# praateekmahajan/moving-mnist-vae

Hardware: AMD Instinct MI355X
Metric: frames/sec/GPU VAE train step, 20×64×64 batch; ELBO vs CPU ref (higher is better)
Workload: dtype bf16; 1 GPU; BASELINE configs[1]: 256 clips x 20 frames x 64x64 per GPU per step (=5120 frames), conv-VAE z=128, Gaussian NLL sigma=0.1 + KL (normal_vae_1_kl_0_mmd), Adam, random-init weights, Bernoulli(0.0521) q=2 labels; parallelism=dp1, rccl_ranks=1, grad_exchange=none, bn=per-rank batch statistics

## Files before the change

include/mmvae.h:

```cpp
#ifndef MMVAE_H_
#define MMVAE_H_

#include <stddef.h>
#include <stdint.h>

#ifdef __cplusplus
extern "C" {
#endif

#if defined(__GNUC__)
#define MMVAE_API __attribute__((visibility("default")))
#else
#define MMVAE_API
#endif

#define MMVAE_OK 0
#define MMVAE_ERR_ARG (-1)
#define MMVAE_ERR_HIP (-2)
#define MMVAE_ERR_WORKSPACE (-3)
#define MMVAE_ERR_UNSUPPORTED (-4)

#define MMVAE_F32 0
#define MMVAE_BF16 1
#define MMVAE_FP8 2
// ... 15 lines not shown
                    int32_t* kind, int64_t* offset);
MMVAE_API size_t mmvae_net_workspace_bytes(mmvae_net* net, int N);

MMVAE_API int mmvae_encoder_fwd(mmvae_net* net, int N, const float* x, const float* params, float* bn_f32, int64_t* bn_i64,
                      void* workspace, size_t workspace_bytes, float* mu, float* logvar, int training, void* stream);
MMVAE_API int mmvae_net_stage_labels(mmvae_net* net, int N, const void* labels, int label_bytes, float mean, float stdv, float* image,
                           void* workspace, size_t workspace_bytes, void* stream);
MMVAE_API int mmvae_encoder_fwd_staged(mmvae_net* net, int N, const float* x, const float* params, float* bn_f32, int64_t* bn_i64,
                             void* workspace, size_t workspace_bytes, float* mu, float* logvar, int training, void* stream);
MMVAE_API int mmvae_encoder_bwd(mmvae_net* net, int N, const float* d_mu, const float* d_logvar, const float* params, float* grads,
                      void* workspace, size_t workspace_bytes, void* stream);
MMVAE_API int mmvae_decoder_fwd(mmvae_net* net, int N, const float* encoding, const float* params, float* bn_f32, int64_t* bn_i64,
                      void* workspace, size_t workspace_bytes, float* recon, int training, void* stream);
MMVAE_API int mmvae_decoder_bwd(mmvae_net* net, int N, const float* d_recon, const float* params, float* grads, void* workspace,
                      size_t workspace_bytes, float* d_encoding , void* stream);
MMVAE_API int mmvae_decoder_bwd_gauss(mmvae_net* net, int N, const float* target, float sigma, float coef, const float* gscale, const float* params,
                            float* grads, void* workspace, size_t workspace_bytes, float* d_enc, void* stream);

MMVAE_API int mmvae_net_defer_join(mmvae_net* net, int enable);
MMVAE_API int mmvae_net_join(mmvae_net* net, void* stream);
MMVAE_API void* mmvae_net_fork(mmvae_net* net, void* stream);
MMVAE_API void* mmvae_net_side_stream(mmvae_net* net);
MMVAE_API int mmvae_net_set_join_grad(mmvae_net* net, int enable);

typedef int (*mmvae_allreduce_fn)(float* buf, int64_t n, void* stream, void* user);
MMVAE_API int mmvae_net_set_sync_bn(mmvae_net* net, mmvae_allreduce_fn fn, void* user, int world);

typedef struct mmvae_comm mmvae_comm;
#define MMVAE_COMM_ID_BYTES 128
MMVAE_API int mmvae_comm_unique_id(void* id_host );
MMVAE_API int mmvae_comm_init(mmvae_comm** out, int world, int rank, const void* id_host);
MMVAE_API int mmvae_comm_allreduce(mmvae_comm* comm, float* buf, int64_t n, void* stream);
MMVAE_API int mmvae_comm_destroy(mmvae_comm* comm);
MMVAE_API int mmvae_net_set_sync_bn_comm(mmvae_net* net, mmvae_comm* comm);
MMVAE_API int mmvae_net_set_sync_bn_comm2(mmvae_net* net, mmvae_comm* comm_main, mmvae_comm* comm_side);

MMVAE_API int mmvae_rsample_fwd(const float* mu, const float* logvar, const float* eps, float* enc, int64_t n, void* stream);
MMVAE_API int mmvae_rsample_bwd(const float* d_enc, const float* logvar, const float* eps, float* d_mu, float* d_logvar, int64_t n,
                      void* stream);
#define MMVAE_SUM_PARTIALS 1025
MMVAE_API int mmvae_kl_fwd(const float* mu, const float* logvar, int64_t n, double* acc, void* stream);
MMVAE_API int mmvae_kl_fwd_ex(const float* mu, const float* logvar, int64_t n, double* acc, double* partials, void* stream);
MMVAE_API int mmvae_kl_bwd(const float* mu, const float* logvar, float coef, const float* gscale, float* d_mu, float* d_logvar, int64_t n,
                 void* stream);
MMVAE_API int mmvae_gauss_nll_fwd(const float* recon, const float* target, int64_t n, float sigma, double* acc, void* stream);
MMVAE_API int mmvae_gauss_nll_fwd_ex(const float* recon, const float* target, int64_t n, float sigma, double* acc, double* partials,
// ... 79 lines not shown
MMVAE_API int mmvae_adam_step(float* params, const float* grads, float* exp_avg, float* exp_avg_sq, int64_t n, float lr, float beta1,
                    float beta2, float eps, float weight_decay, float bc1, float bc2_sqrt, float grad_scale, void* stream);

MMVAE_API int mmvae_adam_step_dev(float* params, const float* grads, float* exp_avg, float* exp_avg_sq, int64_t n, float lr, float beta1,
                        float beta2, float eps, float weight_decay, double* step_dev, float grad_scale, void* stream);

MMVAE_API int mmvae_grad_norm_sq(const float* grads, int64_t n, float grad_scale, double* acc, double* partials, void* stream);

MMVAE_API int mmvae_adam_step_guarded(float* params, const float* grads, float* exp_avg, float* exp_avg_sq, int64_t n, float lr, float beta1,
                            float beta2, float eps, float weight_decay, double* state, double* partials, float grad_scale,
                            float max_norm, void* stream);

MMVAE_API int mmvae_conv2d_fwd(int dtype, int transposed, const void* x, const float* weight, void* y, int N, int H, int W, int Cin, int Cout,
                     int k, int stride, int pad, const float* pro_scale, const float* pro_shift, int pro_relu, float* stats,
                     void* scratch, void* stream);
MMVAE_API int mmvae_conv2d_dgrad(int dtype, int transposed, const void* dy, const float* weight, void* dx, int N, int H, int W, int Cin,
                       int Cout, int k, int stride, int pad, void* scratch, void* stream);
#define MMVAE_DGRAD_EX_W2_OFFSET(numel_w, esize) ((((size_t)(numel_w) * (esize) + 255) / 256) * 256)
#define MMVAE_DGRAD_EX_SCRATCH_BYTES(numel_w, numel_w2, esize) \
  ((numel_w2) > 0 ? MMVAE_DGRAD_EX_W2_OFFSET(numel_w, esize) + (size_t)(numel_w2) * (esize) : (size_t)(numel_w) * (esize))
MMVAE_API int mmvae_conv2d_dgrad_ex(int dtype, int transposed, const void* dy, const float* weight, void* dx, int N, int H, int W, int Cin,
                          int Cout, int k, int stride, int pad, int accumulate, const void* dy2, const float* w2, int C2, void* scratch,
                          void* stream);
#define MMVAE_WGRAD_SCRATCH_BYTES (64u << 20)
MMVAE_API int mmvae_conv2d_wgrad(int dtype, int transposed, const void* x, const void* dy, float* dweight, int N, int H, int W, int Cin,
                       int Cout, int k, int stride, int pad, const float* pro_scale, const float* pro_shift, int pro_relu,
                       void* scratch, void* stream);
MMVAE_API int mmvae_conv2d_wgrad_pair(int dtype, const void* x, const void* dy, const void* dy_shortcut, float* dweight, float* dweight_sc, int N,
                            int H, int W, int Cin, int Cout, const float* pro_scale, const float* pro_shift, int pro_relu, void* scratch,
                            void* stream);
#define MMVAE_BN_SCRATCH_BYTES (16u << 20)
MMVAE_API int mmvae_batchnorm_fwd(int dtype, const void* y, int64_t npix, int C, const float* gamma, const float* beta, float* running_mean,
                        float* running_var, int64_t* nbt, float momentum, float eps, int relu, void* out, float* save_mean, float* save_istd,
                        void* scratch, void* stream);
MMVAE_API int mmvae_batchnorm_bwd(int dtype, const void* dout, const void* y, const void* out, int64_t npix, int C, const float* gamma,
                        const float* save_mean, const float* save_istd, void* dy, float* dgamma, float* dbeta, void* scratch, void* stream);
#define MMVAE_STEM_SCRATCH_BYTES 12800u
MMVAE_API int mmvae_stem_fwd(int dtype, const void* x, const float* weight, void* y, int N, int S, float* stats, void* scratch, void* stream);
MMVAE_API int mmvae_stem_bwd(int dtype, const void* g, const void* y0, const void* x, const float* weight, const float* gamma,
                   const float* bn_scale, const float* bn_shift, const float* save_mean, const float* save_istd, float* dweight,
                   float* dgamma, float* dbeta, int N, int S, void* scratch, void* stream);
MMVAE_API int mmvae_convT_bwd_fused(int dtype, const void* x, const void* dy, const float* weight, float* dweight, void* dx, int N, int H, int W,
                          int Cin, int Cout, int k, int stride, int pad, const float* pro_scale, const float* pro_shift, int pro_relu,
                          const void* x2, const float* w2, float* dw2, void* scratch, void* wscratch, void* stream);
MMVAE_API int mmvae_tail_join_fwd(int dtype, const void* y2, const float* s2, const float* b2, const void* ys, const float* ss, const float* bs,
                        const float* weight, const float* bias, float* r_raw, float* stats, int N, int H, int W, void* stream);
// ... 50 lines not shown
```

moving-mnist-vae_amd/_lib.py:

```python
from __future__ import annotations

import ctypes
import os
from ctypes import POINTER, c_char_p, c_double, c_float, c_int, c_int32, c_int64, c_size_t, c_uint64, c_void_p

import torch

_HERE = os.path.dirname(os.path.abspath(__file__))
LIB_PATH = os.environ.get("MMVAE_LIB_PATH") or os.path.join(_HERE, "libmmvae_hip.so")
_lib = None
ABI_VERSION = 3
SUM_PARTIALS = 1025
BN_SCRATCH_BYTES = 16 << 20
STEM_SCRATCH_BYTES = 12800

P = c_void_p

PROTOTYPES = {
    "mmvae_abi_version": (c_int, []),
    "mmvae_last_error": (c_char_p, []),
    "mmvae_net_create": (c_int, [POINTER(c_void_p), c_int, c_int, c_int, c_int, c_int, c_int]),
    "mmvae_net_create_ex": (c_int, [POINTER(c_void_p), c_int, c_int, c_int, c_int, c_int, c_int, c_int]),
    "mmvae_net_destroy": (None, [P]),
    "mmvae_net_sizes": (c_int, [P, POINTER(c_int64), POINTER(c_int64), POINTER(c_int32), POINTER(c_int64), POINTER(c_int32)]),
    "mmvae_net_num_entries": (c_int, [P]),
    "mmvae_net_entry": (c_int, [P, c_int, c_char_p, c_int, POINTER(c_int32), POINTER(c_int32), POINTER(c_int32), POINTER(c_int64)]),
    "mmvae_net_workspace_bytes": (c_size_t, [P, c_int]),
    "mmvae_encoder_fwd": (c_int, [P, c_int, P, P, P, P, P, c_size_t, P, P, c_int, P]),
    "mmvae_net_stage_labels": (c_int, [P, c_int, P, c_int, c_float, c_float, P, P, c_size_t, P]),
    "mmvae_encoder_fwd_staged": (c_int, [P, c_int, P, P, P, P, P, c_size_t, P, P, c_int, P]),
    "mmvae_encoder_bwd": (c_int, [P, c_int, P, P, P, P, P, c_size_t, P]),
    "mmvae_decoder_fwd": (c_int, [P, c_int, P, P, P, P, P, c_size_t, P, c_int, P]),
    "mmvae_decoder_bwd": (c_int, [P, c_int, P, P, P, P, c_size_t, P, P]),
    "mmvae_decoder_bwd_gauss": (c_int, [P, c_int, P, c_float, c_float, P, P, P, P, c_size_t, P, P]),
    "mmvae_net_defer_join": (c_int, [P, c_int]),
    "mmvae_net_join": (c_int, [P, P]),
    "mmvae_net_fork": (P, [P, P]),
    "mmvae_net_side_stream": (P, [P]),
    "mmvae_net_set_join_grad": (c_int, [P, c_int]),
    "mmvae_net_set_sync_bn": (c_int, [P, P, P, c_int]),
    "mmvae_rsample_fwd": (c_int, [P, P, P, P, c_int64, P]),
    "mmvae_rsample_bwd": (c_int, [P, P, P, P, P, c_int64, P]),
    "mmvae_kl_fwd": (c_int, [P, P, c_int64, P, P]),
    "mmvae_kl_fwd_ex": (c_int, [P, P, c_int64, P, P, P]),
    "mmvae_kl_bwd": (c_int, [P, P, c_float, P, P, P, c_int64, P]),
    "mmvae_gauss_nll_fwd": (c_int, [P, P, c_int64, c_float, P, P]),
    "mmvae_gauss_nll_fwd_ex": (c_int, [P, P, c_int64, c_float, P, P, P]),
    "mmvae_gauss_nll_bwd": (c_int, [P, P, c_int64, c_float, c_float, P, P, P]),
    "mmvae_ce_fwd": (c_int, [P, P, P, c_int, c_int, c_int, P, P]),
    "mmvae_ce_fwd_ex": (c_int, [P, P, P, c_int, c_int, c_int, P, P, P]),
    "mmvae_ce_bwd": (c_int, [P, P, P, c_int, c_int, c_int, c_float, P, P, P]),
    "mmvae_mmd_fwd": (c_int, [P, P, c_int, c_int, P, P, P]),
    "mmvae_mmd_fwd_ex": (c_int, [P, P, c_int, c_int, P, P, P, P]),
    "mmvae_mmd_bwd": (c_int, [P, P, c_int, c_int, c_float, P, P, P]),
    "mmvae_loss_finish": (c_int, [P, P, c_float, c_float, c_float, c_float, P]),
    "mmvae_gauss_nll_per_image": (c_int, [P, P, c_int, c_int64, c_float, P, P]),
    "mmvae_ce_per_image": (c_int, [P, P, P, c_int, c_int, c_int, P, P]),
    "mmvae_kl_per_image": (c_int, [P, P, c_int, c_int, P, P]),
    "mmvae_latent_logratio": (c_int, [P, P, P, c_int, c_int, P, P]),
    "mmvae_iw_bound": (c_int, [P, P, c_int, c_int, P, P]),
    "mmvae_normalise_labels": (c_int, [P, c_int64, c_float, c_float, P, P]),
    "mmvae_quantise_normalise": (c_int, [P, c_int64, P, c_int, c_float, c_float, P, P, P]),
    "mmvae_u8_histogram": (c_int, [P, c_int64, P, c_int64, P, P]),
    "mmvae_kmeans1d_fit": (c_int, [P, c_int, P, P]),
    "mmvae_quantiser_stats": (c_int, [P, P, c_int, P, P, P, P]),
    "mmvae_resample_coeffs": (c_int, [c_int, c_int, POINTER(c_int), P, P]),
    "mmvae_resize_quantise_normalise": (c_int, [P, c_int64, P, c_int, c_int64, c_int, c_int, c_int, c_int, P, P, c_int, P, P, c_int, P, c_int,
                                                c_float, c_float, P, P, P, P]),
    "mmvae_generate_clips": (c_int, [P, c_int64, c_int, P, c_uint64, c_int64, c_int64, c_int, c_int, c_int, P, c_int, c_float, c_float, P, P, P, P]),
    "mmvae_logits_to_labels": (c_int, [P, c_int, c_int, c_int, c_int, P, P, P]),
    "mmvae_panel_sheet": (c_int, [P, c_int, c_int, c_int, P, P]),
    "mmvae_scatter_panel": (c_int, [P, c_int64, c_int, c_int, c_int, P, c_int, c_int, P, P, c_int64, P]),
    "mmvae_latent_stats": (c_int, [P, P, P, c_int, c_int, c_int, P, P]),
    "mmvae_nearest_frames_scratch_bytes": (c_size_t, [c_int, c_int64, c_int, c_int]),
    "mmvae_nearest_frames": (c_int, [P, c_int, P, c_int64, c_int, P, c_int, P, P, P, c_size_t, P]),
    "mmvae_tensor_hist_chunks": (c_int64, [P, c_int, c_int64, P, c_int64]),
    "mmvae_tensor_hist_scratch_bytes": (c_size_t, [c_int, c_int64]),
    "mmvae_tensor_hist": (c_int, [P, c_int64, P, P, c_int, P, P, c_int64, P, P, P, P, P, c_size_t, P]),
    "mmvae_adam_step": (c_int, [P, P, P, P, c_int64, c_float, c_float, c_float, c_float, c_float, c_float, c_float, c_float, P]),
    "mmvae_adam_step_dev": (c_int, [P, P, P, P, c_int64, c_float, c_float, c_float, c_float, c_float, P, c_float, P]),
    "mmvae_grad_norm_sq": (c_int, [P, c_int64, c_float, P, P, P]),
    "mmvae_adam_step_guarded": (c_int, [P, P, P, P, c_int64, c_float, c_float, c_float, c_float, c_float, P, P, c_float, c_float, P]),
    "mmvae_conv2d_fwd": (c_int, [c_int, c_int, P, P, P, c_int, c_int, c_int, c_int, c_int, c_int, c_int, c_int, P, P, c_int, P, P, P]),
    "mmvae_conv2d_dgrad": (c_int, [c_int, c_int, P, P, P, c_int, c_int, c_int, c_int, c_int, c_int, c_int, c_int, P, P]),
    "mmvae_conv2d_dgrad_ex": (c_int, [c_int, c_int, P, P, P, c_int, c_int, c_int, c_int, c_int, c_int, c_int, c_int, c_int, P, P, c_int, P, P]),
    "mmvae_conv2d_wgrad": (c_int, [c_int, c_int, P, P, P, c_int, c_int, c_int, c_int, c_int, c_int, c_int, c_int, P, P, c_int, P, P]),
    "mmvae_conv2d_wgrad_pair": (c_int, [c_int, P, P, P, P, P, c_int, c_int, c_int, c_int, c_int, P, P, c_int, P, P]),
    "mmvae_rbf_kernel": (c_int, [P, P, c_int, c_int, c_int, P, P]),
    "mmvae_comm_unique_id": (c_int, [P]),
    "mmvae_comm_init": (c_int, [POINTER(c_void_p), c_int, c_int, P]),
    "mmvae_comm_allreduce": (c_int, [P, P, c_int64, P]),
    "mmvae_comm_destroy": (c_int, [P]),
    "mmvae_net_set_sync_bn_comm": (c_int, [P, P]),
    "mmvae_net_set_sync_bn_comm2": (c_int, [P, P, P]),
    "mmvae_convT_bwd_fused": (c_int, [c_int, P, P, P, P, P, c_int, c_int, c_int, c_int, c_int, c_int, c_int, c_int, P, P, c_int, P, P, P, P, P, P]),
    "mmvae_batchnorm_fwd": (c_int, [c_int, P, c_int64, c_int, P, P, P, P, P, c_float, c_float, c_int, P, P, P, P, P]),
    "mmvae_batchnorm_bwd": (c_int, [c_int, P, P, P, c_int64, c_int, P, P, P, P, P, P, P, P]),
    "mmvae_stem_fwd": (c_int, [c_int, P, P, P, c_int, c_int, P, P, P]),
    "mmvae_stem_bwd": (c_int, [c_int, P, P, P, P, P, P, P, P, P, P, P, P, c_int, c_int, P, P]),
    "mmvae_tail_join_fwd": (c_int, [c_int, P, P, P, P, P, P, P, P, P, P, c_int, c_int, c_int, P]),
    "mmvae_tail_join_fwd_stream": (c_int, [c_int, P, P, P, P, P, P, P, P, P, P, c_int, c_int, c_int, P]),
    "mmvae_tail_join_bwd_reduce": (c_int, [c_int, P, P, c_int, P, P, P, P, P, P, P, P, c_int, c_int, c_int, P]),
    "mmvae_tail_join_bwd_apply": (c_int, [c_int, P, P, c_int, P, P, P, P, P, P, P, P, P, P, P, P, P, P, c_int, c_int, c_int, P]),
    "mmvae_upblock_bwd_fused": (c_int, [P] * 27 + [c_int, P, P]),
    "mmvae_join_conv1x1_fwd": (c_int, [P, P, P, P, P, P, P, c_int, P, P, P, c_int64, P, P]),
    "mmvae_conv1x1_bwd_fused": (c_int, [P] * 13 + [c_int64, P, P]),
    "mmvae_upblock_tail_fwd": (c_int, [P] * 16 + [c_int, P, P]),
    "mmvae_upblock_tail_fwd_store": (c_int, [P] * 18 + [c_int, P, P]),
# ... 87 lines not shown
```

moving-mnist-vae_amd/csrc/capi.cpp:

```cpp
#include <cstring>
#include <new>

#include "../../include/mmvae.h"
#include "conv_ops.hpp"
#include "pixel_net.hpp"
#include "quantiser_fit.hpp"
#include "resample.hpp"
#include "vae_net.hpp"

namespace mmvae { const char* last_error(); }
using namespace mmvae;

struct mmvae_net { Net* net; };
struct mmvae_comm { Comm* c; };

static inline hipStream_t stream_of(void* s) { return static_cast<hipStream_t>(s); }

extern "C" {

int mmvae_abi_version(void) { return MMVAE_ABI_VERSION; }
const char* mmvae_last_error(void) { return last_error(); }

int mmvae_net_create(mmvae_net** out, int in_channels, int z, int out_channels, int image_size, int need_logvar, int dtype) {
  return mmvae_net_create_ex(out, in_channels, z, out_channels, image_size, need_logvar, dtype, 1);
// ... 84 lines not shown
}

int mmvae_net_defer_join(mmvae_net* n, int enable) {
  if (!n) { set_error("net_defer_join: bad argument"); return MMVAE_ERR_ARG; }
  n->net->set_defer_join(enable != 0);
  return MMVAE_OK;
}
int mmvae_net_join(mmvae_net* n, void* stream) {
  if (!n) { set_error("net_join: bad argument"); return MMVAE_ERR_ARG; }
  return n->net->join(stream_of(stream));
}

void* mmvae_net_fork(mmvae_net* n, void* stream) {
  if (!n) return stream;
  return reinterpret_cast<void*>(n->net->fork(stream_of(stream)));
}

int mmvae_net_set_join_grad(mmvae_net* n, int enable) {
  if (!n) { set_error("net_set_join_grad: bad argument"); return MMVAE_ERR_ARG; }
  n->net->set_join_grad(enable != 0);
  return MMVAE_OK;
}

void* mmvae_net_side_stream(mmvae_net* n) { return n ? reinterpret_cast<void*>(n->net->side()) : nullptr; }

int mmvae_net_set_sync_bn(mmvae_net* n, mmvae_allreduce_fn fn, void* user, int world) {
  if (!n || (fn && world < 1)) { set_error("net_set_sync_bn: bad argument"); return MMVAE_ERR_ARG; }
  n->net->set_sync_bn(reinterpret_cast<mmvae::Net::AllReduceFn>(fn), user, world);
  return MMVAE_OK;
}

int mmvae_comm_unique_id(void* id) {
  if (!id) { set_error("comm_unique_id: bad argument"); return MMVAE_ERR_ARG; }
  return comm_unique_id(id);
}
int mmvae_comm_init(mmvae_comm** out, int world, int rank, const void* id) {
  if (!out || !id || world < 1 || rank < 0 || rank >= world) { set_error("comm_init: bad argument"); return MMVAE_ERR_ARG; }
  mmvae_comm* h = new (std::nothrow) mmvae_comm;
  if (!h) return MMVAE_ERR_ARG;
  h->c = nullptr;
  const int rc = comm_init(&h->c, world, rank, id);
  if (rc < 0) { delete h; return rc; }
  *out = h;
  return MMVAE_OK;
}
int mmvae_comm_allreduce(mmvae_comm* c, float* buf, int64_t n, void* st) {
// ... 287 lines not shown
  if (dy2 && C2 < 1) { set_error("conv2d_dgrad: C2=%d", C2); return MMVAE_ERR_ARG; }
  if (dy2 && !transposed && s == 2 && ((H | W) & 1)) {
    set_error("conv2d_dgrad: a stride-2 second source needs even H and W (%d x %d): its phase (0, 0) is the q grid", H, W); return MMVAE_ERR_ARG;
  }
  const ConvGeom g = geom_for(transposed, Cin, Cout, k, s, p);
  const int Ho = out_size(transposed, H, k, s, p), Wo = out_size(transposed, W, k, s, p);
  char* sc = static_cast<char*>(scratch);
  SecondSrc q;
  if (dy2) {
    const ConvGeom g2 = geom_for(0, Cin, C2, 1, transposed ? 1 : s, 0);
    q.wfrag2 = op_up_layout(dt, g2, H, W, 1).frag;
    void* w2p = sc + MMVAE_DGRAD_EX_W2_OFFSET(numel_w(Cin, Cout, k), dtype_size(dt));
    int rc = op_pack_up(dt, g2, w2, w2p, stream_of(st), 1.f, 0, q.wfrag2); if (rc < 0) return rc;
    q.x2 = dy2; q.w2 = w2p; q.Cin2 = C2;
  }
  if (!transposed) {
    q.wfrag = op_up_layout(dt, g, H, W, accumulate != 0).frag;
    int rc = op_pack_up(dt, g, w, scratch, stream_of(st), 1.f, 0, q.wfrag); if (rc < 0) return rc;
    return op_run_up(dt, g, scratch, N, dy, Ho, Wo, dx, H, W, nullptr, nullptr, 0, nullptr, accumulate != 0, stream_of(st), q);
  }
  q.wfrag = op_down_layout(dt, g, Ho, Wo).frag;
  int rc = op_pack_down(dt, g, w, scratch, stream_of(st), 1.f, 0, q.wfrag); if (rc < 0) return rc;
  return op_run_down(dt, dt, g, scratch, N, dy, Ho, Wo, dx, H, W, nullptr, nullptr, 0, nullptr, accumulate != 0, stream_of(st), q);
}
int mmvae_conv2d_wgrad(int dt, int transposed, const void* x, const void* dy, float* dw, int N, int H, int W, int Cin, int Cout, int k,
                       int s, int p, const float* ps, const float* pb, int relu, void* scratch, void* st) {
  const ConvGeom g = geom_for(transposed, Cin, Cout, k, s, p);
  const int Ho = out_size(transposed, H, k, s, p), Wo = out_size(transposed, W, k, s, p);
  if (!scratch) { set_error("conv2d_wgrad: scratch (MMVAE_WGRAD_SCRATCH_BYTES) required"); return MMVAE_ERR_ARG; }
  static_assert(MMVAE_WGRAD_SCRATCH_BYTES == kWgradScratchBytes, "public scratch size out of sync");
  float* sc = static_cast<float*>(scratch);
  if (!transposed) return op_run_wgrad(dt, g, N, dy, Ho, Wo, nullptr, nullptr, 0, x, H, W, ps, pb, relu, dw, stream_of(st), sc);
  return op_run_wgrad(dt, g, N, x, H, W, ps, pb, relu, dy, Ho, Wo, nullptr, nullptr, 0, dw, stream_of(st), sc);
}
int mmvae_conv2d_wgrad_pair(int dt, const void* x, const void* dy, const void* dy_sc, float* dw, float* dw_sc, int N, int H, int W, int Cin, int Cout,
                            const float* ps, const float* pb, int relu, void* scratch, void* st) {
  if (!scratch || !x || !dy || !dy_sc || !dw || !dw_sc || N < 1) { set_error("conv2d_wgrad_pair: bad argument"); return MMVAE_ERR_ARG; }
  const ConvGeom g = geom_for(0, Cin, Cout, 3, 2, 1), gs = geom_for(0, Cin, Cout, 1, 2, 0);
  const int Ho = out_size(0, H, 3, 2, 1), Wo = out_size(0, W, 3, 2, 1);
  const int rc = op_run_wgrad_pair(dt, g, gs, N, dy, dy_sc, Ho, Wo, x, H, W, ps, pb, relu, dw, dw_sc, stream_of(st), static_cast<float*>(scratch), 1.f, 1.f);
  if (rc == 0) { set_error("conv2d_wgrad_pair: shape not supported (bf16, 32 -> 32 channels, 32x32 -> 16x16)"); return MMVAE_ERR_UNSUPPORTED; }
  return rc < 0 ? rc : MMVAE_OK;
}
int mmvae_convT_bwd_fused(int dt, const void* x, const void* dy, const float* w, float* dw, void* dx, int N, int H, int W, int Cin, int Cout, int k,
                          int s, int p, const float* ps, const float* pb, int relu, const void* x2, const float* w2, float* dw2, void* scratch,
                          void* wscratch, void* st) {
// ... 195 lines not shown
```

moving-mnist-vae_amd/csrc/kernels.hpp:

```cpp
#pragma once
#include "common.hpp"

namespace mmvae {

enum DType : int { DT_F32 = 0, DT_BF16 = 1 };
inline size_t dtype_size(int dt) { return dt == DT_F32 ? 4 : 2; }

struct Tap { int dh, dw; };
constexpr int kMaxTaps = 25;
constexpr int kMaxPhases = 4;
struct Phase { int ph, pw, Hq, Wq, ntaps, tap0; long w_off;  };
struct GatherArgs {
  const void* x; const void* w; void* y;
  const float* pro_scale; const float* pro_shift; int pro_relu;
  const float* bias;
  float* stats;
  int accumulate;
  int N, Hi, Wi, Cin, Ho, Wo, Cout;
  int SI, SO;
  int nphase; Phase phases[kMaxPhases]; Tap taps[kMaxTaps];
  int cin_vecs;
  int x_planar, x_planes;
  int y_planes;
  const void* x2; const void* w2; int Cin2, x2_ph, x2_pw;
// ... 122 lines not shown
  int nw;
  int ntiles;
};
int launch_pos_conv(int K, int S, int P, int up, int HI, int HO, int CIN, const PosArgs* a, hipStream_t s);

struct PackArgs {
  const float* src; void* dst; int cols, K, ntaps; int s_col, s_k; int tap_off[kMaxTaps]; float scale;
  int cols_valid, K_valid;
  int fp8;
  int frag;
};
int launch_pack(int dt, const PackArgs& a, hipStream_t s);
void pack_batch_begin();
int pack_batch_flush(int dt, hipStream_t s);

int launch_stem_im2col(int dt, const void* x, void* col, int N, int H, int W, int Ho, int Wo, hipStream_t s);

bool stem_bwd_fusable(int S);
bool conv3_stream_ok(int dt, int Cin, int Cout, int k, int s, int p, int Hin, int Win);
int launch_conv3_stream_bwd(int dt, const void* dy, const void* w_flipped, void* dx, const void* ym, const float* ms, const float* mb, float* sums,
                            int N, int H, hipStream_t s);
int launch_conv3_stream(int dt, int stride, const void* x, const void* w, const void* wsc, void* y, void* ysc, const float* pro_scale,
                        const float* pro_shift, int pro_relu, float* stats, float* stats_sc, int N, int Ho, hipStream_t s);
bool convT4_stream_ok(int dt, int Cin, int Cout, int k, int s, int p, int Hin, int Win);
int launch_convT4_stream(int dt, const void* x, const void* w_up, void* y, const float* pro_scale, const float* pro_shift, int pro_relu, float* stats,
                         int N, int Hin, hipStream_t s, int f8out = 0);
bool tail_fwd_stream_ok(int dt, int OC, int H, int W);
int launch_tail_fwd_stream(int dt, const void* y2, const float* s2, const float* b2, const void* ys, const float* ss, const float* bs, const float* w,
                           const float* bias, float* r_raw, float* stats, int N, int H, int W, hipStream_t s, int f8in = 0);
bool up5_tail_fwd_ok(int dt, int OC, int C, int Cin, int Hin, int Hout);
int launch_up5_tail_fwd(const void* y1, const float* p1s, const float* p1b, const void* w2_up, const void* xin, const float* pxs, const float* pxb,
                        const void* wu_up, const float* s2, const float* b2, const float* ss, const float* bs, const float* w, const float* bias,
                        float* r_raw, float* stats, int N, hipStream_t s, void* y2 = nullptr, void* ys = nullptr);
bool stem_fwd_stream_ok(int dt, int S);
int launch_stem_fwd_stream(int dt, const void* x, const float* w, void* y, float* stats, int N, int S, hipStream_t s);
int stem_bwd_part_floats();
int launch_stem_gram(int dt, const void* x, float* scratch, long scratch_cap_floats, double* R, int N, int S, int Ho, int Wo, hipStream_t s);
int launch_stem_bwd(int dt, const void* g, const void* y0, const void* x, const float* ms, const float* mb, float* partials,
                    long partials_cap_floats, int N, int S, int Ho, int Wo, hipStream_t s);
bool stem_bwd_dg_ok(int dt, int S);
int launch_stem_bwd_dg(const void* dy1, const void* dys, const void* wd1, const void* wds, const void* y0, const void* x, const float* ms, const float* mb,
                       float* partials, long partials_cap_floats, int N, int S, int Ho, int Wo, hipStream_t s);
int launch_stem_bwd_finalize(const float* partials, int nparts, const double* R, const float* w, const float* global_sums, double count,
                             const float* gamma, const float* mean, const float* istd, float* dgamma, float* dbeta, float* dW, hipStream_t s);

int launch_chan_stats_nhwc(int dt, const void* y, long npix, int C, float* partials, hipStream_t s);
// ... 134 lines not shown
```

moving-mnist-vae_amd/csrc/vae_net.cpp:

```cpp
#include "vae_net.hpp"

#include <algorithm>
#include <cmath>
#include <cstdlib>
#include <cstring>

#include "conv_ops.hpp"

namespace mmvae {

#define MM_TRY(expr)            \
  do {                          \
    int rc__ = (expr);          \
    if (rc__ < 0) return rc__;  \
  } while (0)

static inline long align_up(long v, long a) { return (v + a - 1) / a * a; }
static inline int down_size(int H, int k, int s, int p) { return conv_down_size(H, k, s, p); }

void Net::add_entry(const std::string& name, std::initializer_list<int> shape, int kind, long off) {
  Entry e; e.name = name; e.ndim = (int)shape.size(); e.kind = kind; e.offset = off;
  int i = 0; for (int d : shape) e.shape[i++] = d;
  for (; i < 4; ++i) e.shape[i] = 1;
  entries.push_back(e);
// ... 634 lines not shown
    } else {
      MM_TRY(run_up(ps, B.c2, base + dy2o, B.Hout, B.Wout, base + P.da1, B.Hout, B.Wout, nullptr, nullptr, 0, nullptr, 0, s));
      np = launch_bn_bwd_reduce(dt(), base + P.da1, nullptr, r1.scale, r1.shift, base + B.y1, nullptr, npix, B.C, part, s);
    }
    MM_TRY(np);
    MM_TRY(bn_backward_coefs(ps, B.b1, np, 1, 0, cnt, s));
    MM_TRY(launch_bn_bwd_apply(dt(), base + P.da1, nullptr, r1.scale, r1.shift, base + B.y1, r1.A, r1.B, r1.C, base + dy1o, nullptr, nullptr,
                               nullptr, nullptr, nullptr, npix, B.C, s));
    MM_TRY(side_fork(s));
    int taken = 0;
    if (pair) {
      taken = op_run_wgrad_pair(dt(), geom(B.c1), geom(B.cs), N, base + dy1o, base + dyso, B.Hout, B.Wout, xin, B.Hin, B.Win, xs, xb, 1,
                                grads + B.c1.off, grads + B.cs.off, wsm, ps.wscratch, B.c1.wscale, B.cs.wscale);
      MM_TRY(taken);
      if (!taken) MM_TRY(run_wgrad(ps, B.cs, base + dyso, B.Hout, B.Wout, nullptr, nullptr, xin, B.Hin, B.Win, xs, xb, wsm));
    }
    if (!taken) MM_TRY(run_wgrad(ps, B.c1, base + dy1o, B.Hout, B.Wout, nullptr, nullptr, xin, B.Hin, B.Win, xs, xb, wsm));
    if (late.nparts > 0) MM_TRY(launch_wgrad_reduce(late, wsm));
    MM_TRY(side_mark(i));
    if (i == 0 && stem_dg_fused()) {
      stem_dy1 = dy1o; stem_dys = dyso;
    } else if (B.identity)
      MM_TRY(run_up(ps, B.c1, base + dy1o, B.Hout, B.Wout, base + P.g[cur ^ 1], B.Hin, B.Win, nullptr, nullptr, 0, nullptr, 1, s));
    else
      MM_TRY(run_up(ps, B.c1, base + dy1o, B.Hout, B.Wout, base + P.g[cur ^ 1], B.Hin, B.Win, nullptr, nullptr, 0, nullptr, 0, s, &B.cs,
                    base + dyso));
    cur ^= 1;
  }
  if (stem_bwd_fused()) {
    const long npix = (long)N * H1 * W1;
    const Block& B0 = enc[0];
    const int np = stem_dg_fused()
        ? launch_stem_bwd_dg(base + stem_dy1, base + stem_dys, ps.packed(B0.c1.packU), ps.packed(B0.cs.packU), base + P.y0, base + P.x_t,
                             r0.scale, r0.shift, part, kPartialFloats, N, cfg.S, H1, W1, s)
        : launch_stem_bwd(dt(), base + P.g[cur], base + P.y0, base + P.x_t, r0.scale, r0.shift, part, kPartialFloats, N, cfg.S, H1, W1, s);
    MM_TRY(np);
    const float* gsum = nullptr; double cnt = (double)npix;
    if (sync_bn_on()) {
      float* row = nullptr;
      MM_TRY(sync_rows(ps, part, np, 64, s, &row, stem_bwd_part_floats()));
      gsum = row; cnt *= ar_world_;
    }
    if (side_state_ == 1 && hipStreamWaitEvent(s, gram_ev_, 0) != hipSuccess) { set_error("side stream wait failed"); return MMVAE_ERR_HIP; }
    MM_TRY(launch_stem_bwd_finalize(part, np, reinterpret_cast<const double*>(base + P.stem_R), params + stem.off, gsum, cnt,
                                    params + bn0.g_off, r0.mean, r0.istd, grads + bn0.g_off, grads + bn0.b_off, grads + stem.off, s));
    return side_join(s);
// ... 340 lines not shown
```

moving-mnist-vae_amd/csrc/vae_net.hpp:

```cpp
#pragma once
#include <string>
#include <vector>

#include "comm.hpp"
#include "conv_ops.hpp"
#include "kernels.hpp"

namespace mmvae {

struct NetCfg { int in_ch, z, out_ch, S, need_logvar, dtype, blocks, fp8; };

enum EntryKind : int { EK_PARAM = 0, EK_BN_F32 = 1, EK_BN_I64 = 2 };
struct Entry { std::string name; int ndim; int shape[4]; int kind; long offset; };

struct ConvW { long off; int D0, D1, k, s, p; long packD, packU; int Hl = 0;  bool tr = false;  bool fp8 = false; float wscale = 1.f;
               bool fragD = false, fragU = false;  };
struct Bn {
  long g_off, b_off, rm_off, rv_off; int nbt_idx; int C; long ws;
  enum Row { MEAN, ISTD, SCALE, SHIFT, COEF_A, COEF_B, COEF_C, kRows };
  long row_floats() const { return (C + 3L) / 4 * 4; }
  long row(Row r) const { return ws + r * row_floats(); }
  long scratch_floats() const { return kRows * row_floats(); }
};
struct BnRows { float *mean, *istd, *scale, *shift, *A, *B, *C; };
// ... 108 lines not shown
  int packs_dec_bwd(const Pass& ps, bool need_denc, hipStream_t s);
  int pack_down(const Pass& ps, const ConvW& w, hipStream_t s);
  int pack_up(const Pass& ps, const ConvW& w, hipStream_t s);
  int run_down(const Pass& ps, const ConvW& w, const void* L, int Hl, int Wl, void* S, int Hs, int Ws,
               const float* pro_s, const float* pro_b, int relu, float* stats, int accumulate, int out_dt, hipStream_t s,
               const ConvW* w2 = nullptr, const void* x2 = nullptr);
  int run_up(const Pass& ps, const ConvW& w, const void* S, int Hs, int Ws, void* L, int Hl, int Wl,
             const float* pro_s, const float* pro_b, int relu, float* stats, int accumulate, hipStream_t s,
             const ConvW* w2 = nullptr, const void* x2 = nullptr);
  int run_wgrad(const Pass& ps, const ConvW& w, const void* P, int Hs, int Ws, const float* proP_s, const float* proP_b,
                const void* G, int Hl, int Wl, const float* proG_s, const float* proG_b, hipStream_t s);
  int reduce_wgrad_parts(const Pass& ps, const ConvW& w, const float* parts, int nparts, int ntaps, hipStream_t s);
  bool tail_fwd_fused() const;
  bool stem_bwd_fused() const;
  bool stem_dg_fused() const;
  bool defer_join_ = false;
  int (*ar_fn_)(float*, long long, void*, void*) = nullptr; void* ar_user_ = nullptr; int ar_world_ = 1;
  Comm* comm_ = nullptr; Comm* comm_side_ = nullptr;
  int sync_rows(const Pass& ps, const float* partials, int nparts, int width, hipStream_t s, float** out, int row_stride = 0);
 public:
  void set_defer_join(bool v) { defer_join_ = v; }
  bool join_grad_ = true;
  void set_join_grad(bool v) { join_grad_ = v; }
  typedef int (*AllReduceFn)(float* buf, long long n, void* stream, void* user);
  void set_sync_bn(AllReduceFn fn, void* user, int world) { ar_fn_ = fn; ar_user_ = user; ar_world_ = fn ? world : 1; comm_ = comm_side_ = nullptr; }
  void set_sync_bn_comm(Comm* c, Comm* side = nullptr) { comm_ = c; comm_side_ = c ? side : nullptr; ar_fn_ = nullptr; ar_user_ = nullptr; ar_world_ = c ? comm_world(c) : 1; }
  bool sync_bn_on() const { return ar_fn_ != nullptr || comm_ != nullptr; }
  int join(hipStream_t s) { return side_join(s); }
  hipStream_t side() const { return side_state_ == 1 ? side_ : nullptr; }
  hipStream_t fork(hipStream_t s) { return side_fork(s) == MMVAE_OK ? wgrad_stream(s) : s; }
 private:
  int bn_fwd(const Pass& ps, const Bn& bn, int nparts, double count, hipStream_t s, long part_off = 0, float in_scale = 1.f);
  int fold_bn_eval(const Pass& ps, int which, hipStream_t s);
  bool l1_dgrad_stream() const;
  long l1c2_flip = 0;
  bool eval_folded_ = false;
  bool store8 = false;
  int fill_consts(const Pass& ps, hipStream_t s);
  int bn_backward_coefs(const Pass& ps, const Bn& bn, int nparts, int ny, int which, double count, hipStream_t s, float* dbias_conv = nullptr);
  BnBwdFinalizeArgs bwd_finalize_args(const Pass& ps, const Bn& bn, const float* partials, int nparts, int ny, int which, double count) const;
  int bn_backward_coefs_join(const Pass& ps, const Bn& b2, const Bn& bs, int nparts, double count, hipStream_t s);
};

}
```

Before: 864,800 frames/s.

## Add specialized fused dgrad kernel for encoder entry block with shortcut

Adds a dedicated streaming kernel that computes the input gradient of the encoder's first downsampling residual block (3x3 stride-2 conv plus 1x1 stride-2 shortcut, 32->64 channels on 16x16) in one pass using bf16 MFMA with LDS-resident weights and a ring buffer of dy rows. It replaces the generic run_up dgrad path with the second operand, aiming to cut launch and memory traffic for this layer. It is enabled by default through a new toggle and exposed via a C API. The rounding of the main path to bf16 before adding the shortcut term may shift numerics slightly.

```diff
diff --git a/include/mmvae.h b/include/mmvae.h
--- a/include/mmvae.h
+++ b/include/mmvae.h
@@ -61,6 +61,8 @@
 MMVAE_API void* mmvae_net_fork(mmvae_net* net, void* stream);
 MMVAE_API void* mmvae_net_side_stream(mmvae_net* net);
 MMVAE_API int mmvae_net_set_join_grad(mmvae_net* net, int enable);
+
+MMVAE_API int mmvae_net_set_entry_dgrad(mmvae_net* net, int enable);
 
 typedef int (*mmvae_allreduce_fn)(float* buf, int64_t n, void* stream, void* user);
 MMVAE_API int mmvae_net_set_sync_bn(mmvae_net* net, mmvae_allreduce_fn fn, void* user, int world);
@@ -186,6 +188,8 @@
 MMVAE_API int mmvae_conv2d_dgrad_ex(int dtype, int transposed, const void* dy, const float* weight, void* dx, int N, int H, int W, int Cin,
                           int Cout, int k, int stride, int pad, int accumulate, const void* dy2, const float* w2, int C2, void* scratch,
                           void* stream);
+MMVAE_API int mmvae_entry_dgrad_stream(int dtype, int transposed, const void* dy, const float* weight, const void* dy2, const float* w2, void* dx,
+                             int N, int H, int Cin, int Cout, void* scratch, void* stream);
 #define MMVAE_WGRAD_SCRATCH_BYTES (64u << 20)
 MMVAE_API int mmvae_conv2d_wgrad(int dtype, int transposed, const void* x, const void* dy, float* dweight, int N, int H, int W, int Cin,
                        int Cout, int k, int stride, int pad, const float* pro_scale, const float* pro_shift, int pro_relu,
diff --git a/moving-mnist-vae_amd/_lib.py b/moving-mnist-vae_amd/_lib.py
--- a/moving-mnist-vae_amd/_lib.py
+++ b/moving-mnist-vae_amd/_lib.py
@@ -38,6 +38,7 @@
     "mmvae_net_fork": (P, [P, P]),
     "mmvae_net_side_stream": (P, [P]),
     "mmvae_net_set_join_grad": (c_int, [P, c_int]),
+    "mmvae_net_set_entry_dgrad": (c_int, [P, c_int]),
     "mmvae_net_set_sync_bn": (c_int, [P, P, P, c_int]),
     "mmvae_rsample_fwd": (c_int, [P, P, P, P, c_int64, P]),
     "mmvae_rsample_bwd": (c_int, [P, P, P, P, P, c_int64, P]),
@@ -84,6 +85,7 @@
     "mmvae_conv2d_fwd": (c_int, [c_int, c_int, P, P, P, c_int, c_int, c_int, c_int, c_int, c_int, c_int, c_int, P, P, c_int, P, P, P]),
     "mmvae_conv2d_dgrad": (c_int, [c_int, c_int, P, P, P, c_int, c_int, c_int, c_int, c_int, c_int, c_int, c_int, P, P]),
     "mmvae_conv2d_dgrad_ex": (c_int, [c_int, c_int, P, P, P, c_int, c_int, c_int, c_int, c_int, c_int, c_int, c_int, c_int, P, P, c_int, P, P]),
+    "mmvae_entry_dgrad_stream": (c_int, [c_int, c_int, P, P, P, P, P, c_int, c_int, c_int, c_int, P, P]),
     "mmvae_conv2d_wgrad": (c_int, [c_int, c_int, P, P, P, c_int, c_int, c_int, c_int, c_int, c_int, c_int, c_int, P, P, c_int, P, P]),
     "mmvae_conv2d_wgrad_pair": (c_int, [c_int, P, P, P, P, P, c_int, c_int, c_int, c_int, c_int, P, P, c_int, P, P]),
     "mmvae_rbf_kernel": (c_int, [P, P, c_int, c_int, c_int, P, P]),
diff --git a/moving-mnist-vae_amd/csrc/capi.cpp b/moving-mnist-vae_amd/csrc/capi.cpp
--- a/moving-mnist-vae_amd/csrc/capi.cpp
+++ b/moving-mnist-vae_amd/csrc/capi.cpp
@@ -130,6 +130,12 @@
   return MMVAE_OK;
 }
 
+int mmvae_net_set_entry_dgrad(mmvae_net* n, int enable) {
+  if (!n) { set_error("net_set_entry_dgrad: bad argument"); return MMVAE_ERR_ARG; }
+  n->net->set_entry_dgrad(enable != 0);
+  return MMVAE_OK;
+}
+
 void* mmvae_net_side_stream(mmvae_net* n) { return n ? reinterpret_cast<void*>(n->net->side()) : nullptr; }
 
 int mmvae_net_set_sync_bn(mmvae_net* n, mmvae_allreduce_fn fn, void* user, int world) {
@@ -463,6 +469,22 @@
   q.wfrag = op_down_layout(dt, g, Ho, Wo).frag;
   int rc = op_pack_down(dt, g, w, scratch, stream_of(st), 1.f, 0, q.wfrag); if (rc < 0) return rc;
   return op_run_down(dt, dt, g, scratch, N, dy, Ho, Wo, dx, H, W, nullptr, nullptr, 0, nullptr, accumulate != 0, stream_of(st), q);
+}
+int mmvae_entry_dgrad_stream(int dt, int transposed, const void* dy, const float* w, const void* dy2, const float* w2, void* dx, int N, int H, int Cin,
+                             int Cout, void* scratch, void* st) {
+  if (dt != MMVAE_F32 && dt != MMVAE_BF16) { set_error("entry_dgrad_stream: dtype=%d unsupported", dt); return MMVAE_ERR_ARG; }
+  if (!dy || !w || !dy2 || !w2 || !dx || !scratch || N < 1) { set_error("entry_dgrad_stream: bad argument"); return MMVAE_ERR_ARG; }
+  if (transposed != 0 || !entry_dgrad_stream_ok(dt, transposed, Cin, Cout, H)) {
+    set_error("entry_dgrad_stream: bf16, the encoder entry (32 -> 64 channels on a 16x16 block input); got dtype=%d transposed=%d %d -> %d on %dx%d",
+              dt, transposed, Cin, Cout, H, H);
+    return MMVAE_ERR_UNSUPPORTED;
+  }
+  const ConvGeom g = geom_for(0, Cin, Cout, 3, 2, 1), g2 = geom_for(0, Cin, Cout, 1, 2, 0);
+  const int wfrag = op_up_layout(dt, g, H, H, 0).frag, wfrag2 = op_up_layout(dt, g2, H, H, 1).frag;
+  void* w2p = static_cast<char*>(scratch) + MMVAE_DGRAD_EX_W2_OFFSET(numel_w(Cin, Cout, 3), dtype_size(dt));
+  int rc = op_pack_up(dt, g, w, scratch, stream_of(st), 1.f, 0, wfrag); if (rc < 0) return rc;
+  rc = op_pack_up(dt, g2, w2, w2p, stream_of(st), 1.f, 0, wfrag2); if (rc < 0) return rc;
+  return launch_entry_dgrad_stream(dt, transposed, dy, scratch, wfrag, dy2, w2p, wfrag2, dx, N, stream_of(st));
 }
 int mmvae_conv2d_wgrad(int dt, int transposed, const void* x, const void* dy, float* dw, int N, int H, int W, int Cin, int Cout, int k,
                        int s, int p, const float* ps, const float* pb, int relu, void* scratch, void* st) {
diff --git a/moving-mnist-vae_amd/csrc/conv_dstream.hip b/moving-mnist-vae_amd/csrc/conv_dstream.hip
--- /dev/null
+++ b/moving-mnist-vae_amd/csrc/conv_dstream.hip
@@ -0,0 +1,184 @@
+#include <hip/hip_runtime.h>
+
+#include <string.h>
+
+#include "kernels.hpp"
+#include "tile_common.hpp"
+
+namespace mmvae {
+
+struct EntryDgradArgs {
+  const void* dy; const void* dy2;
+  const void* w; const void* w2;
+  void* dx;
+  int wfrag, wfrag2;
+  int N, HS, nunits;
+};
+
+__device__ __forceinline__ long afrag_elem(int frag, int blk, int chunk, int Ktot, int l) {
+  if (frag) return (((long)blk * (Ktot >> 5) + chunk) * 64 + l) * 8;
+  const int rr = l & 15, g4 = l >> 4;
+  const int col = 32 * (blk >> 1) + 8 * (rr >> 2) + 4 * (blk & 1) + (rr & 3);
+  return (long)col * Ktot + chunk * 32 + 8 * g4;
+}
+
+__device__ __forceinline__ void unit_walk(int nunits, int wv, int& u_first, int& u_step, int& u_end) {
+  const int nblk = gridDim.x;
+  if ((nblk & 7) == 0) {
+    const int per = (nunits + 7) >> 3;
+    const int lo_u = (blockIdx.x & 7) * per;
+    u_first = lo_u + (blockIdx.x >> 3) * 4 + wv; u_step = (nblk >> 3) * 4; u_end = min(nunits, lo_u + per);
+  } else { u_first = blockIdx.x * 4 + wv; u_step = nblk * 4; u_end = nunits; }
+}
+
+constexpr int kDownFrags = 40;
+constexpr int kDownPitch = 144;
+constexpr int kDownRowB = 1408;
+constexpr int kDownSlots = 4;
+
+__global__ __launch_bounds__(256, 2) void entry_dgrad_down_kernel(EntryDgradArgs a) {
+  constexpr int PITCH = kDownPitch, ROWB = kDownRowB, NSLOT = kDownSlots, HQ = 8, ROWG = HQ * 128;
+  extern __shared__ __attribute__((aligned(16))) char smem[];
+  const int t = threadIdx.x, lane = t & 63, wv = __builtin_amdgcn_readfirstlane(t >> 6), gq = lane >> 4, r = lane & 15;
+  char* sWf = smem;
+  char* ring = smem + kDownFrags * 1024 + wv * (NSLOT * ROWB);
+  for (int i = t; i < kDownFrags * 64; i += 256) {
+    const int fi = i >> 6, l = i & 63, f = fi >> 2, h = (fi >> 1) & 1, m = fi & 1;
+    const bf16_t* src;
+    if (f < 9) {
+      const int pbase = f < 1 ? 0 : f < 3 ? 2048 : f < 5 ? 6144 : 10240, ntp = f < 1 ? 1 : f < 5 ? 2 : 4, tp = f < 1 ? 0 : f < 3 ? f - 1 : f < 5 ? f - 3 : f - 5;
+      src = reinterpret_cast<const bf16_t*>(a.w) + pbase + afrag_elem(a.wfrag, m, tp * 2 + h, ntp * 64, l);
+    } else {
+      src = reinterpret_cast<const bf16_t*>(a.w2) + afrag_elem(a.wfrag2, m, h, 64, l);
+    }
+    *reinterpret_cast<Vec16*>(sWf + i * 16) = *reinterpret_cast<const Vec16*>(src);
+  }
+  if (lane < 4 * 8) *reinterpret_cast<Vec16*>(ring + (lane >> 3) * ROWB + 8 * PITCH + (lane & 7) * 16) = Vec16{{0, 0, 0, 0}};
+  __syncthreads();
+
+  int u_first, u_step, u_end;
+  unit_walk(a.nunits, wv, u_first, u_step, u_end);
+  const int nstrips = (HQ / 2) / a.HS;
+  const int nq = a.HS + 1;
+  const char* DY = reinterpret_cast<const char*>(a.dy);
+  const char* DS = reinterpret_cast<const char*>(a.dy2);
+  u32x4_t dv[2], sv[2] = {(u32x4_t){0, 0, 0, 0}, (u32x4_t){0, 0, 0, 0}};
+  auto issue = [&](int u, int q) {
+    const int n = u / nstrips, s0 = (u - n * nstrips) * a.HS;
+    const int row0 = 2 * (s0 + q) - 1;
+#pragma unroll
+    for (int k = 0; k < 2; ++k) {
+      const int row = row0 + k;
+      dv[k] = (u32x4_t){0, 0, 0, 0};
+      if (row >= 0 && row < HQ && (q > 0 || k == 1)) dv[k] = *reinterpret_cast<const u32x4_t*>(DY + ((long)n * HQ + row) * ROWG + lane * 16);
+    }
+    if (q >= 1) {
+      const char* p = DS + ((long)n * HQ + 2 * (s0 + q - 1)) * ROWG + r * 128 + gq * 16;
+      sv[0] = *reinterpret_cast<const u32x4_t*>(p);
+      sv[1] = *reinterpret_cast<const u32x4_t*>(p + 64);
+    }
+  };
+  auto commit = [&](int u, int q) {
+    const int n = u / nstrips, s0 = (u - n * nstrips) * a.HS;
+    const int row0 = 2 * (s0 + q) - 1;
+#pragma unroll
+    for (int k = 0; k < 2; ++k)
+      *reinterpret_cast<u32x4_t*>(ring + ((row0 + k + NSLOT) & (NSLOT - 1)) * ROWB + (lane >> 3) * PITCH + (lane & 7) * 16) = dv[k];
+    (void)n;
+  };
+  auto wf = [&](int f, int h, int m) { return *reinterpret_cast<const Vec16*>(sWf + ((((f * 2 + h) * 2 + m) * 64) + lane) * 16); };
+
+  const int j = r >> 3, wq = r & 7;
+  int u = u_first, q = 0;
+  if (u < u_end) issue(u, 0);
+  while (u < u_end) {
+    commit(u, q);
+    const Vec16 s0v = __builtin_bit_cast(Vec16, sv[0]), s1v = __builtin_bit_cast(Vec16, sv[1]);
+    int un = u, qn = q + 1;
+    if (qn == nq) { un = u + u_step; qn = 0; }
+    if (un < u_end) issue(un, qn);
+    __builtin_amdgcn_sched_barrier(0);
+    if (q >= 1) {
+      const int n = u / nstrips, s = (u - n * nstrips) * a.HS + q - 1;
+      Vec16 b[2][2][2];
+#pragma unroll
+      for (int dh = 0; dh < 2; ++dh) {
+        const char* rp = ring + ((2 * s + j + dh) & (NSLOT - 1)) * ROWB + wq * PITCH + gq * 16;
+#pragma unroll
+        for (int dw = 0; dw < 2; ++dw)
+#pragma unroll
+          for (int h = 0; h < 2; ++h) b[dh][dw][h] = *reinterpret_cast<const Vec16*>(rp + dw * PITCH + h * 64);
+      }
+      f32x4 acc[4][2];
+#pragma unroll
+      for (int p = 0; p < 4; ++p) { acc[p][0] = (f32x4){0, 0, 0, 0}; acc[p][1] = (f32x4){0, 0, 0, 0}; }
+      f32x4 asc[2];
+#pragma unroll
+      for (int m = 0; m < 2; ++m) {
+        asc[m] = (f32x4){0, 0, 0, 0};
+#pragma unroll
+        for (int h = 0; h < 2; ++h) acc[0][m] = mma_bf16(wf(0, h, m), b[0][0][h], acc[0][m]);
+#pragma unroll
+        for (int h = 0; h < 2; ++h) acc[1][m] = mma_bf16(wf(1, h, m), b[0][1][h], acc[1][m]);
+#pragma unroll
+        for (int h = 0; h < 2; ++h) acc[1][m] = mma_bf16(wf(2, h, m), b[0][0][h], acc[1][m]);
+#pragma unroll
+        for (int h = 0; h < 2; ++h) acc[2][m] = mma_bf16(wf(3, h, m), b[1][0][h], acc[2][m]);
+#pragma unroll
+        for (int h = 0; h < 2; ++h) acc[2][m] = mma_bf16(wf(4, h, m), b[0][0][h], acc[2][m]);
+#pragma unroll
+        for (int h = 0; h < 2; ++h) acc[3][m] = mma_bf16(wf(5, h, m), b[1][1][h], acc[3][m]);
+#pragma unroll
+        for (int h = 0; h < 2; ++h) acc[3][m] = mma_bf16(wf(6, h, m), b[1][0][h], acc[3][m]);
+#pragma unroll
+        for (int h = 0; h < 2; ++h) acc[3][m] = mma_bf16(wf(7, h, m), b[0][1][h], acc[3][m]);
+#pragma unroll
+        for (int h = 0; h < 2; ++h) acc[3][m] = mma_bf16(wf(8, h, m), b[0][0][h], acc[3][m]);
+        asc[m] = mma_bf16(wf(9, 0, m), s0v, asc[m]);
+        asc[m] = mma_bf16(wf(9, 1, m), s1v, asc[m]);
+      }
+      bf16_t* G = reinterpret_cast<bf16_t*>(a.dx) + ((((long)n * 16 + 2 * (2 * s + j)) * 16) + 2 * wq) * 32 + 8 * gq;
+#pragma unroll
+      for (int p = 0; p < 4; ++p) {
+        float v[8] = {acc[p][0][0], acc[p][0][1], acc[p][0][2], acc[p][0][3], acc[p][1][0], acc[p][1][1], acc[p][1][2], acc[p][1][3]};
+        if (p == 0) {
+          const float sc[8] = {asc[0][0], asc[0][1], asc[0][2], asc[0][3], asc[1][0], asc[1][1], asc[1][2], asc[1][3]};
+          float m1[8];
+          Elem<bf16_t>::unpack(Elem<bf16_t>::pack(v), m1);
+#pragma unroll
+          for (int jj = 0; jj < 8; ++jj) v[jj] = sc[jj] + m1[jj];
+        }
+        dstore8<bf16_t>(G + ((p >> 1) * 16 + (p & 1)) * 32, v, false);
+      }
+    }
+    __builtin_amdgcn_sched_barrier(0);
+    u = un; q = qn;
+  }
+}
+
+bool entry_dgrad_stream_ok(int dt, int transposed, int Cin, int Cout, int Hin) {
+  return dt == DT_BF16 && !transposed && Cin == 32 && Cout == 64 && Hin == 16;
+}
+
+int launch_entry_dgrad_stream(int dt, int transposed, const void* dy, const void* w, int wfrag, const void* dy2, const void* w2, int wfrag2, void* dx,
+                              int N, hipStream_t s) {
+  if (dt != DT_BF16 || transposed) { set_error("entry_dgrad_stream: bf16, the encoder entry (32 -> 64 channels, 16x16 block input)"); return MMVAE_ERR_UNSUPPORTED; }
+  if (!dy || !w || !dy2 || !w2 || !dx || N < 1) { set_error("entry_dgrad_stream: bad argument"); return MMVAE_ERR_ARG; }
+  EntryDgradArgs a; memset(&a, 0, sizeof(a));
+  a.dy = dy; a.dy2 = dy2; a.w = w; a.w2 = w2; a.dx = dx; a.wfrag = wfrag; a.wfrag2 = wfrag2; a.N = N;
+  a.HS = 2; a.nunits = N * (4 / a.HS);
+  int gx = 512;
+  while (gx > 8 && (long)gx * 4 > a.nunits) gx -= 8;
+  const size_t lds = kDownFrags * 1024 + 4 * (size_t)(kDownSlots * kDownRowB);
+  static bool attr_set = false;
+  if (!attr_set) {
+    const hipError_t e = hipFuncSetAttribute(reinterpret_cast<const void*>(&entry_dgrad_down_kernel), hipFuncAttributeMaxDynamicSharedMemorySize, 160 * 1024);
+    if (e != hipSuccess) { set_error("entry_dgrad_stream: hipFuncSetAttribute: %s", hipGetErrorString(e)); return MMVAE_ERR_HIP; }
+    attr_set = true;
+  }
+  hipLaunchKernelGGL(entry_dgrad_down_kernel, dim3(gx), dim3(256), lds, s, a);
+  note_launch_bytes((double)N * (2.0 * 8 * 8 * 64 + 16.0 * 16 * 32) * 2.0);
+  return check_launch("entry_dgrad_stream");
+}
+
+}
diff --git a/moving-mnist-vae_amd/csrc/kernels.hpp b/moving-mnist-vae_amd/csrc/kernels.hpp
--- a/moving-mnist-vae_amd/csrc/kernels.hpp
+++ b/moving-mnist-vae_amd/csrc/kernels.hpp
@@ -168,6 +168,9 @@
                             int N, int H, hipStream_t s);
 int launch_conv3_stream(int dt, int stride, const void* x, const void* w, const void* wsc, void* y, void* ysc, const float* pro_scale,
                         const float* pro_shift, int pro_relu, float* stats, float* stats_sc, int N, int Ho, hipStream_t s);
+bool entry_dgrad_stream_ok(int dt, int transposed, int Cin, int Cout, int Hin);
+int launch_entry_dgrad_stream(int dt, int transposed, const void* dy, const void* w, int wfrag, const void* dy2, const void* w2, int wfrag2, void* dx,
+                              int N, hipStream_t s);
 bool convT4_stream_ok(int dt, int Cin, int Cout, int k, int s, int p, int Hin, int Win);
 int launch_convT4_stream(int dt, const void* x, const void* w_up, void* y, const float* pro_scale, const float* pro_shift, int pro_relu, float* stats,
                          int N, int Hin, hipStream_t s, int f8out = 0);
diff --git a/moving-mnist-vae_amd/csrc/vae_net.cpp b/moving-mnist-vae_amd/csrc/vae_net.cpp
--- a/moving-mnist-vae_amd/csrc/vae_net.cpp
+++ b/moving-mnist-vae_amd/csrc/vae_net.cpp
@@ -680,6 +680,10 @@
       stem_dy1 = dy1o; stem_dys = dyso;
     } else if (B.identity)
       MM_TRY(run_up(ps, B.c1, base + dy1o, B.Hout, B.Wout, base + P.g[cur ^ 1], B.Hin, B.Win, nullptr, nullptr, 0, nullptr, 1, s));
+    else if (entry_dgrad_ && !B.c1.fp8 && !B.cs.fp8 && B.c1.k == 3 && B.c1.s == 2 && B.c1.p == 1 && B.cs.k == 1 && B.cs.s == 2 && B.cs.p == 0 &&
+             B.Hin == B.Win && entry_dgrad_stream_ok(dt(), 0, B.Cin, B.C, B.Hin))
+      MM_TRY(launch_entry_dgrad_stream(dt(), 0, base + dy1o, ps.packed(B.c1.packU), B.c1.fragU, base + dyso, ps.packed(B.cs.packU), B.cs.fragU,
+                                       base + P.g[cur ^ 1], N, s));
     else
       MM_TRY(run_up(ps, B.c1, base + dy1o, B.Hout, B.Wout, base + P.g[cur ^ 1], B.Hin, B.Win, nullptr, nullptr, 0, nullptr, 0, s, &B.cs,
                     base + dyso));
diff --git a/moving-mnist-vae_amd/csrc/vae_net.hpp b/moving-mnist-vae_amd/csrc/vae_net.hpp
--- a/moving-mnist-vae_amd/csrc/vae_net.hpp
+++ b/moving-mnist-vae_amd/csrc/vae_net.hpp
@@ -154,6 +154,8 @@
   void set_defer_join(bool v) { defer_join_ = v; }
   bool join_grad_ = true;
   void set_join_grad(bool v) { join_grad_ = v; }
+  bool entry_dgrad_ = true;
+  void set_entry_dgrad(bool v) { entry_dgrad_ = v; }
   typedef int (*AllReduceFn)(float* buf, long long n, void* stream, void* user);
   void set_sync_bn(AllReduceFn fn, void* user, int world) { ar_fn_ = fn; ar_user_ = user; ar_world_ = fn ? world : 1; comm_ = comm_side_ = nullptr; }
   void set_sync_bn_comm(Comm* c, Comm* side = nullptr) { comm_ = c; comm_side_ = c ? side : nullptr; ar_fn_ = nullptr; ar_user_ = nullptr; ar_world_ = c ? comm_world(c) : 1; }
```

Result: no change. 872,500 frames/s (median of 6 runs) (+0.9%).
